# calvinmccarter/cocoa

Hardware: AMD Instinct MI355X
Metric: CoCoA+ SVM wall-clock to duality gap 1e-4; coord updates/s at 1/2/4/8 GPUs (higher is better)
Workload: dtype f64

## Files before the change

### cocoa_amd/csrc/engine.hip

```cpp
#include <hip/hip_runtime.h>

#include <sys/stat.h>
#include <unistd.h>

#include <algorithm>
#include <cerrno>
#include <cmath>
#include <cstdio>
#include <cstdlib>
#include <cstring>
#include <mutex>
#include <string>
#include <thread>
#include <vector>

#include "../../include/cocoa_capi.h"
#include "comm.h"
#include "common.h"
#include "jrandom.h"
#include "kernels.h"

using namespace cocoa;

static std::mutex g_err_mu;
// ... 192 lines not shown
    int64_t xw_stride = 0;
    hipEvent_t e_w = nullptr, e_xw = nullptr;
    bool e_w_rec = false;
    void gram_quiesce() {
        if (gstream) HIPCHK(hipStreamSynchronize(gstream));
        pre_t = -1;
    }
    hipStream_t estream = nullptr;
    hipEvent_t e_round = nullptr, e_done = nullptr;
    bool eval_pending = false;
    bool inl_pending = false;
    bool inl_since_round = false;
    bool inl_ranks = false;
    int64_t n_test_glob = -1;
    hipEvent_t e_inl = nullptr;
    cocoa_eval_result eval_held{};
    bool eval_fired = false;
    DevBuf w_snap, alpha_snap, eval_part2, eval_out2;
    DevBuf eval_cnt, eval_cnt2;
    void eval_quiesce();
    DevBuf plan_beg, plan_z, plan_zc, plan_y, plan_q, plan_xw;
    DevBuf plan_beg2, plan_z2, plan_zc2, plan_y2, plan_q2;
    bool pre_plan = false;
    DevBuf row_xw;
    bool xw_cached = false;
    Csr hot_tr, cold_tr, warm_tr;
    DevBuf hot_tiles, cold_tiles, warm_tiles, row_base;
    int64_t n_hot_tiles = 0, n_cold_tiles = 0, n_warm_tiles = 0;
    bool split_ready = false;
    Csr hot_te, cold_te;
    DevBuf hot_t_tiles, cold_t_tiles;
    int64_t n_hot_t_tiles = 0, n_cold_t_tiles = 0;
    bool te_split = false;
    DevBuf csc_ptr, csc_row, csc_val, csc_tiles, row_cnt, row_c;
    int64_t n_csc_tiles = 0;
    bool csc_ready = false;
    bool mbsgd_pull = false;
    int32_t max_z = 0;

    bool stats = false;
    uint32_t stats_mask = ~0u;
    struct Pending {
        int kid;
        hipEvent_t a, b;
    };
    std::vector<Pending> pending;
    std::vector<hipEvent_t> ev_pool;
    double tot_ms[COCOA_K_COUNT] = {0};
    int64_t cnt[COCOA_K_COUNT] = {0};

    hipEvent_t get_ev() {
        if (!ev_pool.empty()) {
            hipEvent_t e = ev_pool.back();
            ev_pool.pop_back();
            return e;
        }
        hipEvent_t e;
        HIPCHK(hipEventCreate(&e));
        return e;
    }
    template <class F>
    void timed(int kid, F&& f) {
        timed_on(stream, kid, f);
    }
    template <class F>
    void timed_on(hipStream_t st, int kid, F&& f) {
// ... 689 lines not shown
            return x.first < y.first;
        });
        int64_t a = hp[(size_t)r], b = cp[(size_t)r];
        for (const auto& cvp : tmp) {
            if (cvp.first < kEvalHot) {
                hc[(size_t)a] = (uint16_t)cvp.first;
                hv[(size_t)a++] = cvp.second;
            } else {
                cc[(size_t)b] = cvp.first;
                cv[(size_t)b++] = cvp.second;
            }
        }
    }
    ctx->hot_te = Csr{};
    ctx->cold_te = Csr{};
    ctx->hot_te.n = ctx->cold_te.n = n;
    ctx->hot_te.nnz = nh;
    ctx->cold_te.nnz = nc;
    upload(ctx->hot_te.row_ptr, hp.data(), sizeof(int64_t) * (size_t)(n + 1), s);
    upload_padded(ctx->hot_te.col16, hc.data(), sizeof(uint16_t) * (size_t)nh, s);
    upload_padded(ctx->hot_te.val, hv.data(), sizeof(double) * (size_t)nh, s);
    upload(ctx->cold_te.row_ptr, cp.data(), sizeof(int64_t) * (size_t)(n + 1), s);
    upload_padded(ctx->cold_te.col, cc.data(), sizeof(int32_t) * (size_t)nc, s);
    upload_col16(ctx->cold_te.col16, cc, nc, ctx->d, s);
    upload_padded(ctx->cold_te.val, cv.data(), sizeof(double) * (size_t)nc, s);
    int hcap = kEvalTile, ccap = kEvalTile;
    eval_split_tiles(&hcap, &ccap);
    ctx->n_hot_t_tiles = make_tiles(hp.data(), n, ctx->hot_t_tiles, s, hcap);
    ctx->n_cold_t_tiles = make_tiles(cp.data(), n, ctx->cold_t_tiles, s, ccap);
    ctx->row_base.alloc(sizeof(double) * (size_t)(ctx->tr.n + n));
    ctx->te_split = ctx->n_hot_t_tiles > 0;
}

static void set_train_impl(cocoa_ctx* ctx, bool dense_in, int32_t num_parts, const int64_t* part_ptr,
                           const int64_t* row_ptr, const int32_t* col, const double* val, const double* y,
                           int64_t n_rows, int32_t num_features, int32_t part_begin, int32_t num_parts_global) {
    require(dense_in || col != nullptr, COCOA_E_ARG, "cocoa_set_train: null column array");
    ctx->gram_quiesce();
    ctx->eval_quiesce();
    require(num_parts >= 1 && part_ptr && row_ptr && y && n_rows >= 0 && num_features >= 1, COCOA_E_ARG,
            "cocoa_set_train: bad argument");
    require(part_begin >= 0 && num_parts_global >= part_begin + num_parts, COCOA_E_ARG,
            "cocoa_set_train: bad partition range");
    require(part_ptr[0] == 0 && part_ptr[num_parts] == n_rows, COCOA_E_ARG, "part_ptr must span [0, n_rows]");
    for (int k = 0; k < num_parts; ++k) require(part_ptr[k + 1] >= part_ptr[k], COCOA_E_ARG, "part_ptr not monotone");
    if (!dense_in) check_csr(row_ptr, col, n_rows, num_features);
    const int64_t nnz = row_ptr[n_rows];
    require(val != nullptr || nnz == 0, COCOA_E_ARG, "cocoa_set_train: null value array");
    ctx->tr_dense = dense_in ? n_rows >= 1 : is_dense(row_ptr, col, n_rows, num_features);
    ctx->csc_ready = false;
    ctx->te_split = false;
    if (ctx->has_test) {
        ctx->has_test = false;
        ctx->te_dense = false;
        ctx->te.n = ctx->te.nnz = 0;
        ctx->n_t_tiles = 0;
        ctx->n_test_glob = -1;
    }
    ctx->K_loc = num_parts;
    ctx->K_glob = num_parts_global;
    ctx->part_begin = part_begin;
    ctx->d = num_features;
    ctx->tr.n = n_rows;
    ctx->tr.nnz = nnz;
    ctx->h_part_ptr.assign(part_ptr, part_ptr + num_parts + 1);
    ctx->max_nl = 0;
// ... 89 lines not shown
    ctx->tr.col_lazy = dense_in;
    if (dense_in) {
        ctx->tr.col.free();
        ctx->tr.col16.free();
    } else {
        upload_padded(ctx->tr.col, pcol.data(), sizeof(int32_t) * (size_t)nnz, s);
        upload_col16(ctx->tr.col16, pcol, nnz, num_features, s);
    }
    upload_padded(ctx->tr.val, split_classes ? pval.data() : val, sizeof(double) * (size_t)nnz, s);
    if (split_classes)
        upload(ctx->row_zc, zcv.data(), sizeof(int32_t) * kGramRuns * (size_t)n_rows, s);
    else
        ctx->row_zc.free();
    upload(ctx->tr.y, y, sizeof(double) * (size_t)n_rows, s);
    upload(ctx->sqn, sq.data(), sizeof(double) * (size_t)n_rows, s);
    upload(ctx->rowflags, fl.data(), (size_t)n_rows, s);
    upload(ctx->part_ptr, part_ptr, sizeof(int64_t) * (size_t)(num_parts + 1), s);
    ctx->n_tiles = make_tiles(row_ptr, n_rows, ctx->tiles, s, eval_tile_entries(num_features));
    if (!dense_in && !ctx->tr_dense)
        build_eval_split(ctx, row_ptr, pcol, split_classes ? pval.data() : val, n_rows, num_features, s);
    else
        ctx->split_ready = false;
    if (dense_in) {
        ctx->compact_ready = false;
        ctx->priv_ready = false;
        ctx->col_local.free();
        ctx->fptr.free();
        ctx->fpos.free();
    } else {
        build_compact(ctx, row_ptr, pcol.data(), split_classes ? pval.data() : val);
    }
    HIPCHK(hipStreamSynchronize(s));
    ctx->inited = false;
}

extern "C" int cocoa_set_test(cocoa_ctx* ctx, const int64_t* row_ptr, const int32_t* col, const double* val,
                              const double* y, int64_t n_rows) {
    CAPI_BEGIN(ctx)
    require(col != nullptr || (row_ptr && n_rows >= 0 && row_ptr[n_rows] == 0), COCOA_E_ARG,
            "cocoa_set_test: null column array");
    static const int32_t no_col = 0;
    if (!col) col = &no_col;
    if (ctx->is_group()) {
        group_set_test(ctx, false, row_ptr, col, val, y, n_rows);
        return COCOA_OK;
    }
    set_test_impl(ctx, false, row_ptr, col, val, y, n_rows);
    CAPI_END(ctx)
}

static void set_test_impl(cocoa_ctx* ctx, bool dense_in, const int64_t* row_ptr, const int32_t* col,
                          const double* val, const double* y, int64_t n_rows) {
    require(dense_in || col != nullptr, COCOA_E_ARG, "cocoa_set_test: null column array");
    ctx->eval_quiesce();
    ctx->te_split = false;
    require(ctx->d > 0, COCOA_E_STATE, "cocoa_set_test: call cocoa_set_train first");
    require(row_ptr && y && n_rows >= 0, COCOA_E_ARG, "cocoa_set_test: bad argument");
    if (!dense_in) check_csr(row_ptr, col, n_rows, ctx->d);
    const int64_t nnz = row_ptr[n_rows];
    require(val != nullptr || nnz == 0, COCOA_E_ARG, "cocoa_set_test: null value array");
    hipStream_t s = ctx->stream;
    ctx->te_dense = dense_in ? n_rows >= 1 : is_dense(row_ptr, col, n_rows, ctx->d);
    ctx->te.n = n_rows;
    ctx->te.nnz = nnz;
    upload(ctx->te.row_ptr, row_ptr, sizeof(int64_t) * (size_t)(n_rows + 1), s);
    ctx->te.col_lazy = dense_in;
    if (dense_in) {
        ctx->te.col.free();
        ctx->te.col16.free();
    } else {
        std::vector<int32_t> pcol((size_t)std::max<int64_t>(nnz, 1));
        for (int64_t q = 0; q < nnz; ++q) pcol[(size_t)q] = ctx->perm[(size_t)col[q]];
        upload_padded(ctx->te.col, pcol.data(), sizeof(int32_t) * (size_t)nnz, s);
        upload_col16(ctx->te.col16, pcol, nnz, ctx->d, s);
        build_test_split(ctx, row_ptr, pcol, val, n_rows, s);
    }
    upload_padded(ctx->te.val, val, sizeof(double) * (size_t)nnz, s);
    upload(ctx->te.y, y, sizeof(double) * (size_t)n_rows, s);
    ctx->n_t_tiles = make_tiles(row_ptr, n_rows, ctx->t_tiles, s, eval_tile_entries(ctx->d));
    HIPCHK(hipStreamSynchronize(s));
    ctx->has_test = true;
    ctx->n_test_glob = -1;
    if (ctx->inited) {
        const size_t rows = (size_t)(ctx->tr.n + ctx->te.n);
        ctx->row_scratch.alloc(sizeof(double) * std::max<size_t>(rows, 1));
    }
}

static bool is_sdca(int m) { return m == COCOA_METHOD_COCOA_PLUS || m == COCOA_METHOD_COCOA || m == COCOA_METHOD_MBCD; }
static int solver_mode(int m) {
    return m == COCOA_METHOD_COCOA_PLUS ? MODE_PLUS : m == COCOA_METHOD_COCOA ? MODE_COCOA : MODE_MBCD;
}
static int32_t wrap32(int64_t x) { return (int32_t)(uint32_t)(uint64_t)x; }

static void plan_solver(cocoa_ctx* c, int64_t vec_len, bool need_prod = true) {
    SolverArgs& a = c->sa;
    size_t off = 0;
    const size_t vec_bytes = align16(sizeof(double) * (size_t)vec_len);
    int ncu = 256;
    (void)hipDeviceGetAttribute(&ncu, hipDeviceAttributeMultiprocessorCount, c->device);
    const int want = (int)std::min<int64_t>(4, std::max<int64_t>(1, ((int64_t)c->K_loc + ncu - 1) / std::max(ncu, 1)));
    const size_t budget = want > 1 ? (kLdsMax / (size_t)want) & ~(size_t)1023 : kLdsMax;
    const double zavg = c->tr.n ? (double)c->tr.nnz / (double)c->tr.n : 0.0;
    size_t cap = zavg * 4 > (double)kStreamCap ? 2 * (size_t)kStreamCap : (size_t)kStreamCap;
    auto fixed_for = [&](size_t cp) {
        return 2 * align16(cp * 4) + 2 * align16(cp * 8) + 2 * align16(sizeof(BatchMeta)) +
               (need_prod ? align16(cp * 8) : 0) + align16(sizeof(double) * kRegChunks * 64);
    };
    while (want > 1 && cap > 512 && fixed_for(cap) > budget) cap /= 2;
    if (const char* e = std::getenv("COCOA_CHAIN_CAP"))
        cap = std::max<size_t>(256, std::min<size_t>(cap, (size_t)std::atoi(e)));
    const size_t fixed = fixed_for(cap);
    size_t avail = (want > 1 ? budget : kLdsMax) - std::min(fixed, budget);
    c->vec_lds = is_sdca(c->method) && vec_bytes <= avail && want == 1;
// ... 955 lines not shown
            e.t_val = ctx->cold_te.val.as<double>();
            e.t_tiles = ctx->cold_t_tiles.as<int64_t>();
            e.n_t_tiles = ctx->n_cold_t_tiles;
            e.th_row_ptr = ctx->hot_te.row_ptr.as<int64_t>();
            e.th_col16 = ctx->hot_te.col16.as<uint16_t>();
            e.th_val = ctx->hot_te.val.as<double>();
            e.th_tiles = ctx->hot_t_tiles.as<int64_t>();
            e.n_th_tiles = ctx->n_hot_t_tiles;
        }
        if (ctx->n_warm_tiles > 0) {
            e.m_row_ptr = ctx->warm_tr.row_ptr.as<int64_t>();
            e.m_col16 = ctx->warm_tr.col16.as<uint16_t>();
            e.m_val = ctx->warm_tr.val.as<double>();
            e.m_tiles = ctx->warm_tiles.as<int64_t>();
            e.n_m_tiles = ctx->n_warm_tiles;
        }
    }
    ctx->timed_on(st, COCOA_K_EVAL, [&] {
        if (ctx->strict)
            launch_eval_strict(e, st);
        else {
            e.row_xw = async ? nullptr : ctx->row_xw.as<double>();
            if (dense_eval) {
                launch_eval_dense(e, st);
            } else {
                DevBuf& cnt = async ? ctx->eval_cnt2 : ctx->eval_cnt;
                if (!cnt.p) cnt.alloc_zero(sizeof(unsigned), st);
                e.counter = cnt.as<unsigned>();
                e.out_host = to_host ? ctx->h_eval + (async ? 4 : 0) : nullptr;
                if (to_host && gram_status) {
                    e.status = async ? ctx->status_snap.as<int>() : ctx->status.as<int>();
                    e.status_host = (int*)(ctx->h_eval + (async ? 10 : 9));
                }
                host_done = launch_eval_fast(e, eval_fast_blocks(e.n_tiles, e.n_t_tiles), st);
            }
            ctx->xw_cached = !async;
        }
    });
    if (to_host && gram_status && !host_done)
        HIPCHK(hipMemcpyAsync(ctx->h_eval + (async ? 10 : 9), async ? ctx->status_snap.p : ctx->status.p, sizeof(int),
                              hipMemcpyDeviceToHost, st));
    ctx->status_slot[async ? 1 : 0] = to_host && gram_status;
    if (async) {
        if (!host_done)
            HIPCHK(hipMemcpyAsync(ctx->h_eval + 4, ctx->eval_out2.p, 4 * sizeof(double), hipMemcpyDeviceToHost, st));
        HIPCHK(hipEventRecord(ctx->e_done, st));
    } else if (!host_done && to_host) {
        HIPCHK(hipMemcpyAsync(ctx->h_eval, ctx->eval_out.p, 4 * sizeof(double), hipMemcpyDeviceToHost, st));
    }
}

static void check_status_slot(cocoa_ctx* ctx, int which) {
    if (!ctx->status_slot[which]) return;
    ctx->status_slot[which] = false;
    if (*(volatile int*)(ctx->h_eval + 9 + which) != 0)
        throw Error(COCOA_E_HIP, "local solver: a hand-off between the solver's waves timed out (launch aborted)");
}

struct EvalLocal {
    double hinge, alpha_sum, w2, err, n_test;
};

static EvalLocal eval_collect(cocoa_ctx* ctx) {
    HIPCHK(hipStreamSynchronize(ctx->stream));
    check_status(ctx);
    return EvalLocal{ctx->h_eval[0], ctx->h_eval[1], ctx->h_eval[2], ctx->h_eval[3],
                     (double)(ctx->has_test ? ctx->te.n : 0)};
// ... 1117 lines not shown
```

### cocoa_amd/csrc/kernels.h

```cpp
#pragma once
#include <hip/hip_runtime.h>

#include <cstdint>

namespace cocoa {

enum SolverMode : int { MODE_PLUS = 0, MODE_COCOA = 1, MODE_MBCD = 2, MODE_LSGD = 3 };

constexpr int kWave = 64;
#ifndef COCOA_RUNS
#define COCOA_RUNS 8
#endif
constexpr int kGramRuns = COCOA_RUNS;
static_assert(kGramRuns == 4 || kGramRuns == 8, "column runs");
constexpr int kGramClasses = 2;
constexpr int kProfStride = 128;
constexpr int kMetaSteps = 64;
#ifndef COCOA_REG_CHUNKS
#define COCOA_REG_CHUNKS 4
#endif
constexpr int kRegChunks = COCOA_REG_CHUNKS;
constexpr int short_row_chunks(int mode, bool strict) {
    return (strict || mode == 1) ? kRegChunks : (mode == 2 ? (kRegChunks < 2 ? kRegChunks : 2) : (kRegChunks < 3 ? kRegChunks : 3));
}
// ... 141 lines not shown
};
constexpr int kXbR = 8;

struct XwArgs {
    const int64_t* part_ptr;
    const int32_t* samples;
    const int64_t* row_ptr;
    const int32_t* col;
    const double* val;
    const double* w;
    double* xw;
    int32_t* flag;
    int64_t stride;
    int32_t K, H, nbatch, epoch;
};

struct DenseArgs {
    const double* X;
    const int64_t* part_ptr;
    const int32_t* samples;
    const double* plan_y;
    const double* plan_q;
    double* alpha;
    double* dw;
    const double* w;
    int64_t d;
    int32_t H;
    int32_t proj;
    double lam_n, inv_lam_n;
    double sigma;
    double scaling;
};

struct EvalArgs {
    const int64_t* row_ptr;
    const int32_t* col;
    const double* val;
    const double* y;
    const double* alpha;
    int64_t n;
    const int64_t* t_row_ptr;
    const int32_t* t_col;
    const double* t_val;
    const double* t_y;
    int64_t n_test;
    const double* w;
    int64_t d;
    const int64_t* part_ptr;
    const int32_t* perm;
    int32_t K;
    int32_t pad;
    const int64_t* tiles;
    int64_t n_tiles;
    const int64_t* t_tiles;
    int64_t n_t_tiles;
    double* partials;
    double* out;
    double* row_scratch;
    double* row_xw;
    const uint16_t* col16;
    const uint16_t* t_col16;
    unsigned* counter;
    double* out_host;
    const int* status;
    int* status_host;
    const int64_t* h_row_ptr;
    const uint16_t* h_col16;
    const double* h_val;
    const int64_t* h_tiles;
    int64_t n_h_tiles;
    double* row_base;
    const int64_t* m_row_ptr;
    const uint16_t* m_col16;
    const double* m_val;
    const int64_t* m_tiles;
    int64_t n_m_tiles;
    const int64_t* th_row_ptr;
    const uint16_t* th_col16;
    const double* th_val;
    const int64_t* th_tiles;
    int64_t n_th_tiles;
};
constexpr int kEvalHot = 4096;
constexpr int kEvalWarm = 65536;
void eval_split_tiles(int* hot_cap, int* cold_cap);

void launch_solver_fast(int mode, bool vec_lds, bool alpha_lds, const SolverArgs& a, int grid, size_t lds,
                        hipStream_t s);
bool launch_eval_fast(const EvalArgs& a, int blocks, hipStream_t s);
int eval_fast_blocks(int64_t n, int64_t n_test);
constexpr int64_t kEvalWideD = 65536;
int eval_tile_entries(int64_t d);
void launch_plan_fast(const PlanArgs& a, hipStream_t s);
size_t gram_solver_lds(int64_t d, int32_t* hot, bool mirror = false);
void launch_gram(const GramArgs& a, hipStream_t s);
size_t gram_seq_lds();
int gram_window_batches();
bool gram_seq_supported();
void launch_xw_produce(const XwArgs& a, hipStream_t s);
void launch_xw_gather(const int64_t* part_ptr, const int32_t* samples, int32_t H, int64_t steps,
                      const double* row_xw, double* xw, hipStream_t s);
void launch_solver_gram(int mode, const GramSolverArgs& a, int grid, hipStream_t s);
bool dense_solver_fits(int64_t d, int64_t max_nl);
bool dense_eval_fits(int64_t d);
void launch_solver_dense(int mode, const DenseArgs& a, int grid, int64_t max_nl, hipStream_t s);
void launch_eval_dense(const EvalArgs& a, hipStream_t s);

void launch_plan_strict(const PlanArgs& a, hipStream_t s);
void launch_solver_strict(int mode, bool vec_lds, bool alpha_lds, const SolverArgs& a, int grid, size_t lds,
                          hipStream_t s);
void launch_eval_strict(const EvalArgs& a, hipStream_t s);
void launch_sampler(const int64_t* part_ptr, int32_t K, int32_t seed, int32_t H, int32_t* samples,
                    const uint64_t* jump_tab, hipStream_t s);
void launch_zero(double* p, int64_t n, int blocks, hipStream_t s);
void launch_dense_cols(int32_t* col, uint16_t* col16, int64_t nnz, int32_t d, hipStream_t s);
void launch_sum_slices(double* own, const double* stage, int32_t n, int32_t r, int64_t len, hipStream_t s);
void launch_fold(const double* dw, int32_t K, int64_t d, double* dw_sum, double* w, double mult, bool apply,
                 const int32_t* inv, bool zero, hipStream_t s, const double* init = nullptr);
constexpr int64_t kFoldJ = 4096;
constexpr int64_t kFoldItem = 32768;
struct FoldTail {
    const uint32_t* tbnd;
    const uint16_t* tcol16;
// ... 35 lines not shown
```

### cocoa_amd/csrc/kernels_fast.hip

```cpp
#include <algorithm>
#include <cstdlib>

#include "kernels.h"
#include "plan_impl.h"
#include "solver_dense.h"
#include "solver_gram.h"
#include "solver_impl.h"
#include "wave.h"

namespace cocoa {

void launch_solver_fast(int mode, bool vec_lds, bool alpha_lds, const SolverArgs& a, int grid, size_t lds,
                        hipStream_t s) {
    launch_solver_impl<false>(mode, vec_lds, alpha_lds, a, grid, lds, s);
}

void launch_plan_fast(const PlanArgs& a, hipStream_t s) { launch_plan_impl<false>(a, s); }

size_t gram_solver_lds(int64_t d, int32_t* hot, bool mirror) {
    constexpr size_t kLds = 160 * 1024;
    const size_t st = mirror ? sizeof(GramSolverLdsT<kGramRuns / 2>) : sizeof(GramSolverLdsT<kGramClasses>);
    const size_t base = (st + 15) & ~(size_t)15;
    const int64_t h = std::max<int64_t>(0, std::min<int64_t>(d, (int64_t)((kLds - base) / sizeof(double)) & ~(int64_t)63));
    if (hot) *hot = (int32_t)h;
// ... 112 lines not shown
    if (!gram_hot_lds() || g.hot == 0) {
        g.mirror = 0;
        lds = (sizeof(GramSolverLdsT<kGramClasses>) + 15) & ~(size_t)15;
        g.hot = 0;
        if (mode == MODE_PLUS) launch_sg<MODE_PLUS, false>(g, grid, lds, s);
        else if (mode == MODE_COCOA) launch_sg<MODE_COCOA, false>(g, grid, lds, s);
        else if (mode == MODE_LSGD) launch_sg3<MODE_LSGD, false, false>(g, grid, lds, s);
        else launch_sg<MODE_MBCD, false>(g, grid, lds, s);
        return;
    }
    if (mode == MODE_PLUS) launch_sg<MODE_PLUS, true>(g, grid, lds, s);
    else if (mode == MODE_COCOA) launch_sg<MODE_COCOA, true>(g, grid, lds, s);
    else if (mode == MODE_LSGD) launch_sg3<MODE_LSGD, true, false>(g, grid, lds, s);
    else launch_sg<MODE_MBCD, true>(g, grid, lds, s);
}

typedef int32_t i32x4 __attribute__((ext_vector_type(4)));
typedef double f64x2 __attribute__((ext_vector_type(2)));

template <int BLOCK>
__device__ __forceinline__ double block_sum_n(double v, double* red) {
    v = wave_sum(v);
    __syncthreads();
    if ((threadIdx.x & 63) == 0) red[threadIdx.x >> 6] = v;
    __syncthreads();
    double s = 0.0;
    for (int i = 0; i < BLOCK / 64; ++i) s += red[i];
    return s;
}

typedef uint16_t u16x4 __attribute__((ext_vector_type(4)));

template <bool C16>
__device__ __forceinline__ i32x4 load_cols(const int32_t* c32, const uint16_t* c16, int64_t k) {
    if (C16) {
        const u16x4 v = __builtin_nontemporal_load((const u16x4*)(c16 + k));
        return i32x4{(int32_t)v.x, (int32_t)v.y, (int32_t)v.z, (int32_t)v.w};
    }
    return __builtin_nontemporal_load((const i32x4*)(c32 + k));
}

typedef __attribute__((address_space(1))) const double gdouble;
typedef __attribute__((address_space(3))) const double ldouble;
template <int HOT>
__device__ __forceinline__ double w_at(const double* w, const double* whot, int32_t c) {
    double x;
    if (HOT > 0 && c < HOT)
        x = ((ldouble*)whot)[c];
    else
        x = ((gdouble*)w)[c];
    return x;
}

__device__ __forceinline__ void eval_reduce(const double* partials, int blocks, double* out, double* out_host,
                                            double (*red)[4], bool sc1) {
    const int tid = threadIdx.x;
    double v[4] = {0, 0, 0, 0};
    if (tid < 256)
        for (int b = tid; b < blocks; b += 256)
            for (int i = 0; i < 4; ++i) {
                double* q = const_cast<double*>(partials) + (size_t)b * 4 + i;
                v[i] += sc1 ? __hip_atomic_load(q, __ATOMIC_RELAXED, __HIP_MEMORY_SCOPE_AGENT) : *q;
            }
    for (int i = 0; i < 4; ++i) {
        const double s = wave_sum(v[i]);
        if ((tid & 63) == 0 && tid < 256) red[i][tid >> 6] = s;
    }
    __syncthreads();
    if (tid < 4) {
        const double r = ((red[tid][0] + red[tid][1]) + red[tid][2]) + red[tid][3];
        out[tid] = r;
        if (out_host) __hip_atomic_store(out_host + tid, r, __ATOMIC_RELAXED, __HIP_MEMORY_SCOPE_SYSTEM);
    }
}

template <int TILE, int BLOCK, bool C16, int DIAGW = 0, int HOT = 0, bool BASE = false>
__global__ __launch_bounds__(BLOCK) void eval_stream_kernel(EvalArgs a) {
    constexpr int UNITS = TILE / (4 * BLOCK);
    __shared__ double prod[TILE + 4];
    __shared__ uint16_t roff[TILE + 2];
    __shared__ double red[BLOCK / 64];
    __shared__ double whot[HOT > 0 ? HOT : 1];
    __shared__ double yl[kEvalRows];
    __shared__ double bl[BASE ? kEvalRows : 1];
    const int tid = threadIdx.x;
    if (HOT > 0) {
        const int32_t h = (int32_t)min<int64_t>(HOT, a.d);
        for (int32_t j = tid; j < h; j += BLOCK) whot[j] = a.w[j];
        __syncthreads();
    }
    const int sub = tid & 15, grp = tid >> 4;
    double hinge = 0.0, err = 0.0;
    const int64_t ntiles = a.n_tiles + a.n_t_tiles;
    for (int64_t t = blockIdx.x; t < ntiles; t += gridDim.x) {
        const bool test = t >= a.n_tiles;
        const int64_t tt = test ? t - a.n_tiles : t;
        const int64_t* tl = test ? a.t_tiles : a.tiles;
        const int64_t* te = tl + (test ? a.n_t_tiles : a.n_tiles) + 1;
        const int64_t* rp = test ? a.t_row_ptr : a.row_ptr;
        const int32_t* cl = test ? a.t_col : a.col;
        const uint16_t* cl16 = test ? a.t_col16 : a.col16;
        const double* vl = test ? a.t_val : a.val;
        const double* yy = test ? a.t_y : a.y;
        const int64_t r0 = tl[tt], r1 = tl[tt + 1];
        const int64_t e0 = te[tt], e1 = te[tt + 1];
        const int64_t T = e1 - e0;
        const bool has_base = BASE && (!test || a.n_th_tiles > 0);
        const double* rb = test ? a.row_base + a.n : a.row_base;
        if (T > TILE) {
            double acc = 0.0;
            for (int64_t q = e0 + tid; q < e1; q += BLOCK) acc += vl[q] * a.w[cl[q]];
            const double dot = block_sum_n<BLOCK>(acc, red) + (has_base ? rb[r0] : 0.0);
            if (tid == 0) {
                if (!test) {
                    hinge += jmax(1 - yy[r0] * dot, 0.0);
                    if (a.row_xw) a.row_xw[r0] = dot;
                } else {
                    err += (dot * yy[r0] > 0) ? 0.0 : 1.0;
                }
            }
            continue;
        }
        const int nr = (int)(r1 - r0);
        for (int i = tid; i <= nr; i += BLOCK) {
            roff[i] = (uint16_t)(rp[r0 + i] - e0);
            if (i < nr) {
                yl[i] = yy[r0 + i];
                if (has_base) bl[i] = rb[r0 + i];
            }
        }
        const int64_t base = e0 & ~(int64_t)3;
        const int sh = (int)(e0 - base);
        const int64_t span = e1 - base;
        i32x4 c[UNITS + 1];
        f64x2 v0[UNITS + 1], v1[UNITS + 1];
#pragma unroll
        for (int u = 0; u <= UNITS; ++u) {
            const int64_t k = 4 * ((int64_t)u * BLOCK + tid);
            c[u] = i32x4{0, 0, 0, 0};
            v0[u] = f64x2{0.0, 0.0};
            v1[u] = v0[u];
            if (k < span) {
                c[u] = load_cols<C16>(cl, cl16, base + k);
                if (DIAGW == 1) c[u] &= 4095;
                if (DIAGW == 2) c[u] &= 0;
                v0[u] = __builtin_nontemporal_load((const f64x2*)(vl + base + k));
                v1[u] = __builtin_nontemporal_load((const f64x2*)(vl + base + k + 2));
            }
        }
#pragma unroll
        for (int u = 0; u <= UNITS; ++u) {
            const int64_t k = 4 * ((int64_t)u * BLOCK + tid);
            if (k < span) {
                *(f64x2*)(prod + k) = f64x2{v0[u].x * w_at<HOT>(a.w, whot, c[u].x), v0[u].y * w_at<HOT>(a.w, whot, c[u].y)};
                *(f64x2*)(prod + k + 2) = f64x2{v1[u].x * w_at<HOT>(a.w, whot, c[u].z), v1[u].y * w_at<HOT>(a.w, whot, c[u].w)};
            }
        }
        __syncthreads();
        for (int r = grp; r < nr; r += BLOCK / 16) {
            const int b = roff[r] + sh, e = roff[r + 1] + sh;
            double acc = 0.0;
            for (int q = b + sub; q < e; q += 16) acc += prod[q];
            double dot = row16_sum(acc);
            if (sub == 0) {
                if (has_base) dot += bl[r];
                if (!test) {
                    hinge += jmax(1 - yl[r] * dot, 0.0);
                    if (a.row_xw) a.row_xw[r0 + r] = dot;
                } else {
                    err += (dot * yl[r] > 0) ? 0.0 : 1.0;
                }
            }
        }
        __syncthreads();
    }
    const int64_t gt = (int64_t)blockIdx.x * BLOCK + tid;
    const int64_t gs = (int64_t)gridDim.x * BLOCK;
    double al = 0.0, w2 = 0.0;
    for (int64_t i = gt; i < a.n; i += gs) al += a.alpha[i];
    for (int64_t j = gt; j < a.d; j += gs) w2 += a.w[j] * a.w[j];
    const double s0 = block_sum_n<BLOCK>(hinge, red);
    const double s1 = block_sum_n<BLOCK>(al, red);
    const double s2 = block_sum_n<BLOCK>(w2, red);
    const double s3 = block_sum_n<BLOCK>(err, red);
// ... 62 lines not shown
        if (sub == 0) {
            if (!test) {
                hinge += jmax(1 - a.y[rr] * dot, 0.0);
                if (a.row_xw) a.row_xw[rr] = dot;
            } else {
                err += (dot * a.t_y[rr] > 0) ? 0.0 : 1.0;
            }
        }
    }
    const int64_t gt = (int64_t)blockIdx.x * 256 + tid, gs = (int64_t)gridDim.x * 256;
    double al = 0.0, w2 = 0.0;
    for (int64_t i = gt; i < a.n; i += gs) al += a.alpha[i];
    for (int64_t j = gt; j < a.d; j += gs) w2 += a.w[j] * a.w[j];
    const double s0 = block_sum_n<256>(hinge, red);
    const double s1 = block_sum_n<256>(al, red);
    const double s2 = block_sum_n<256>(w2, red);
    const double s3 = block_sum_n<256>(err, red);
    if (tid == 0) {
        double* p = a.partials + (size_t)blockIdx.x * 4;
        p[0] = s0;
        p[1] = s1;
        p[2] = s2;
        p[3] = s3;
    }
}

#endif

__global__ __launch_bounds__(256) void eval_final_kernel(const double* partials, int blocks, double* out) {
    __shared__ double red[4][4];
    eval_reduce(partials, blocks, out, nullptr, red, false);
}

int eval_fast_blocks(int64_t n_tiles, int64_t n_t_tiles) {
    int64_t b = n_tiles + n_t_tiles;
    if (b > 256 * 3) b = 256 * 3;
    return (int)(b < 1 ? 1 : b);
}

#ifdef COCOA_DIAG
static int eval_variant() {
    static int v = -1;
    if (v < 0) {
        const char* e = getenv("COCOA_EVAL_VARIANT");
        v = e ? atoi(e) : 0;
    }
    return v;
}
int eval_tile_entries(int64_t d) {
    if (const char* e = getenv("COCOA_EVAL_TILE")) return atoi(e) == 2048 ? 2048 : kEvalTile;
    if (eval_variant() >= 6 && eval_variant() <= 9) return 2048;
    return d > kEvalWideD ? 2048 : kEvalTile;
}

static bool launch_eval_diag(const EvalArgs& a, bool c16, hipStream_t s) {
    const int v = eval_variant();
    if (v == 8 || v == 9) {
        const int64_t nt = a.n_tiles + a.n_t_tiles;
        if (v == 8) {
            const int nb = (int)std::max<int64_t>(1, std::min<int64_t>(nt, 1024));
            if (c16) eval_stream_kernel<2048, 512, true><<<nb, 512, 0, s>>>(a);
            else eval_stream_kernel<2048, 512, false><<<nb, 512, 0, s>>>(a);
            eval_final_kernel<<<1, 256, 0, s>>>(a.partials, nb, a.out);
        } else {
            const int nb = (int)std::max<int64_t>(1, std::min<int64_t>(nt, 2048));
            if (c16) eval_stream_kernel<2048, 256, true><<<nb, 256, 0, s>>>(a);
            else eval_stream_kernel<2048, 256, false><<<nb, 256, 0, s>>>(a);
            eval_final_kernel<<<1, 256, 0, s>>>(a.partials, nb, a.out);
        }
        return true;
    }
#define COCOA_EVAL_C16(...)                          \
    do {                                             \
// ... 18 lines not shown
            const int n2 = (int)std::min<int64_t>(a.n_tiles + a.n_t_tiles, 512);
            COCOA_EVAL_C16((eval_stream_kernel<2048, 512, C, 0, 8192><<<n2, 512, 0, s>>>(a)));
            eval_final_kernel<<<1, 256, 0, s>>>(a.partials, n2, a.out);
        }
        return true;
    }
    if (v == 3 || v == 4) {
        const int nb = eval_fast_blocks(a.n_tiles, a.n_t_tiles);
        if (v == 3) COCOA_EVAL_C16((eval_stream_kernel<kEvalTile, 512, C, 1><<<nb, 512, 0, s>>>(a)));
        else COCOA_EVAL_C16((eval_stream_kernel<kEvalTile, 512, C, 2><<<nb, 512, 0, s>>>(a)));
        eval_final_kernel<<<1, 256, 0, s>>>(a.partials, nb, a.out);
        return true;
    }
#undef COCOA_EVAL_C16
    if (v == 1 || v == 2) {
        const int nb = 2048;
        if (v == 1) {
            if (c16) eval_rows_kernel<8, true><<<nb, 256, 0, s>>>(a);
            else eval_rows_kernel<8, false><<<nb, 256, 0, s>>>(a);
        } else {
            if (c16) eval_rows_kernel<4, true><<<nb, 256, 0, s>>>(a);
            else eval_rows_kernel<4, false><<<nb, 256, 0, s>>>(a);
        }
        eval_final_kernel<<<1, 256, 0, s>>>(a.partials, nb, a.out);
        return true;
    }
    return false;
}
#else
int eval_tile_entries(int64_t d) { return d > kEvalWideD ? 2048 : kEvalTile; }
#endif

template <int TILE, int BLOCK, int HOT, bool WARM = false>
__global__ __launch_bounds__(BLOCK) void eval_hot_kernel(EvalArgs a) {
    constexpr int UNITS = TILE / (4 * BLOCK);
    __shared__ double prod[TILE + 4];
    __shared__ uint16_t roff[TILE + 2];
    __shared__ double red[BLOCK / 64];
    __shared__ double whot[WARM ? 1 : HOT];
    __shared__ double bl[WARM ? kEvalRows : 1];
    const int tid = threadIdx.x;
    if (!WARM) {
        const int32_t h = (int32_t)min<int64_t>(HOT, a.d);
        for (int32_t j = tid; j < HOT; j += BLOCK) whot[j] = j < h ? a.w[j] : 0.0;
        __syncthreads();
    }
    const gdouble* wm = (const gdouble*)(a.w + kEvalHot);
    auto w_of = [&](int32_t c) -> double { return WARM ? wm[c] : whot[c]; };
    const int sub = tid & 15, grp = tid >> 4;
    const int64_t nt = WARM ? a.n_m_tiles : a.n_h_tiles;
    const int64_t ntt = WARM ? 0 : a.n_th_tiles;
    for (int64_t t = blockIdx.x; t < nt + ntt; t += gridDim.x) {
        const bool test = t >= nt;
        const int64_t tt = test ? t - nt : t;
        const int64_t* tl = test ? a.th_tiles : WARM ? a.m_tiles : a.h_tiles;
        const int64_t* te = tl + (test ? ntt : nt) + 1;
        const int64_t* rp = test ? a.th_row_ptr : WARM ? a.m_row_ptr : a.h_row_ptr;
        const uint16_t* cl = test ? a.th_col16 : WARM ? a.m_col16 : a.h_col16;
        const double* vl = test ? a.th_val : WARM ? a.m_val : a.h_val;
        double* rb = test ? a.row_base + a.n : a.row_base;
        const int64_t r0 = tl[tt], r1 = tl[tt + 1];
        const int64_t e0 = te[tt], e1 = te[tt + 1];
        const int64_t T = e1 - e0;
        if (T > TILE) {
            double acc = 0.0;
            for (int64_t q = e0 + tid; q < e1; q += BLOCK) acc += vl[q] * w_of(cl[q]);
            const double dot = block_sum_n<BLOCK>(acc, red);
            if (tid == 0) rb[r0] = WARM ? rb[r0] + dot : dot;
            continue;
        }
        const int nr = (int)(r1 - r0);
        for (int i = tid; i <= nr; i += BLOCK) {
            roff[i] = (uint16_t)(rp[r0 + i] - e0);
            if (WARM && i < nr) bl[i] = rb[r0 + i];
        }
        const int64_t base = e0 & ~(int64_t)3;
        const int sh = (int)(e0 - base);
        const int64_t span = e1 - base;
        i32x4 c[UNITS + 1];
        f64x2 v0[UNITS + 1], v1[UNITS + 1];
#pragma unroll
        for (int u = 0; u <= UNITS; ++u) {
            const int64_t k = 4 * ((int64_t)u * BLOCK + tid);
            c[u] = i32x4{0, 0, 0, 0};
            v0[u] = f64x2{0.0, 0.0};
            v1[u] = v0[u];
            if (k < span) {
                c[u] = load_cols<true>(nullptr, cl, base + k);
                v0[u] = __builtin_nontemporal_load((const f64x2*)(vl + base + k));
                v1[u] = __builtin_nontemporal_load((const f64x2*)(vl + base + k + 2));
            }
        }
#pragma unroll
        for (int u = 0; u <= UNITS; ++u) {
            const int64_t k = 4 * ((int64_t)u * BLOCK + tid);
            if (k < span) {
                *(f64x2*)(prod + k) = f64x2{v0[u].x * w_of(c[u].x), v0[u].y * w_of(c[u].y)};
                *(f64x2*)(prod + k + 2) = f64x2{v1[u].x * w_of(c[u].z), v1[u].y * w_of(c[u].w)};
            }
        }
        __syncthreads();
        for (int r = grp; r < nr; r += BLOCK / 16) {
            const int b = roff[r] + sh, e = roff[r + 1] + sh;
            double acc = 0.0;
            for (int q = b + sub; q < e; q += 16) acc += prod[q];
            const double dot = row16_sum(acc);
            if (sub == 0) rb[r0 + r] = WARM ? bl[r] + dot : dot;
        }
        __syncthreads();
    }
}

#ifndef COCOA_HOT_TILE
#define COCOA_HOT_TILE 4096
#endif
#ifndef COCOA_HOT_BLOCK
#define COCOA_HOT_BLOCK 1024
#endif
#ifndef COCOA_HOT_WGS
#define COCOA_HOT_WGS 2
#endif
#ifndef COCOA_COLD_TILE
#define COCOA_COLD_TILE 4096
#endif
#ifndef COCOA_COLD_BLOCK
#define COCOA_COLD_BLOCK 512
#endif
void eval_split_tiles(int* hot_cap, int* cold_cap) {
    *hot_cap = COCOA_HOT_TILE;
    *cold_cap = COCOA_COLD_TILE;
}

template <typename F>
static int resident_grid(F kernel, int threads, int want) {
    int per_cu = 0, dev = 0, cus = 256;
    (void)hipGetDevice(&dev);
    (void)hipDeviceGetAttribute(&cus, hipDeviceAttributeMultiprocessorCount, dev);
    if (hipOccupancyMaxActiveBlocksPerMultiprocessor(&per_cu, kernel, threads, 0) != hipSuccess || per_cu < 1) {
        (void)hipGetLastError();
        return want;
    }
    return std::max(1, std::min(want, per_cu * cus));
}

static bool launch_eval_split(const EvalArgs& a, int blocks, hipStream_t s) {
    const bool c16 = a.col16 && (a.n_test == 0 || a.t_col16);
    const int hb = (int)std::max<int64_t>(1, std::min<int64_t>(a.n_h_tiles + a.n_th_tiles, 256 * COCOA_HOT_WGS));
    eval_hot_kernel<COCOA_HOT_TILE, COCOA_HOT_BLOCK, kEvalHot><<<hb, COCOA_HOT_BLOCK, 0, s>>>(a);
    if (a.n_m_tiles > 0) {
        const int mb = resident_grid(eval_hot_kernel<COCOA_HOT_TILE, COCOA_HOT_BLOCK, kEvalHot, true>, COCOA_HOT_BLOCK,
                                     (int)std::max<int64_t>(1, std::min<int64_t>(a.n_m_tiles, 256 * 8)));
        eval_hot_kernel<COCOA_HOT_TILE, COCOA_HOT_BLOCK, kEvalHot, true><<<mb, COCOA_HOT_BLOCK, 0, s>>>(a);
    }
    if (c16) {
        blocks = resident_grid(eval_stream_kernel<COCOA_COLD_TILE, COCOA_COLD_BLOCK, true, 0, 0, true>, COCOA_COLD_BLOCK,
                               blocks);
        eval_stream_kernel<COCOA_COLD_TILE, COCOA_COLD_BLOCK, true, 0, 0, true><<<blocks, COCOA_COLD_BLOCK, 0, s>>>(a);
    } else {
        blocks = resident_grid(eval_stream_kernel<COCOA_COLD_TILE, COCOA_COLD_BLOCK, false, 0, 0, true>,
                               COCOA_COLD_BLOCK, blocks);
        eval_stream_kernel<COCOA_COLD_TILE, COCOA_COLD_BLOCK, false, 0, 0, true><<<blocks, COCOA_COLD_BLOCK, 0, s>>>(a);
    }
    if (!a.counter) eval_final_kernel<<<1, 256, 0, s>>>(a.partials, blocks, a.out);
    return a.counter && a.out_host;
}

bool launch_eval_fast(const EvalArgs& a, int blocks, hipStream_t s) {
    if (a.row_base) return launch_eval_split(a, blocks, s);
    const bool c16 = a.col16 && (a.n_test == 0 || a.t_col16);
#ifdef COCOA_DIAG
    EvalArgs u = a;
    u.counter = nullptr;
    if (launch_eval_diag(u, c16, s)) return false;
#endif
    if (c16) {
        blocks = resident_grid(eval_stream_kernel<kEvalTile, 512, true>, 512, blocks);
        eval_stream_kernel<kEvalTile, 512, true><<<blocks, 512, 0, s>>>(a);
    } else if (a.d > kEvalWideD) {
        blocks = resident_grid(eval_stream_kernel<2048, 512, false, 0, 4096>, 512, blocks);
        eval_stream_kernel<2048, 512, false, 0, 4096><<<blocks, 512, 0, s>>>(a);
    } else {
        blocks = resident_grid(eval_stream_kernel<kEvalTile, 512, false>, 512, blocks);
        eval_stream_kernel<kEvalTile, 512, false><<<blocks, 512, 0, s>>>(a);
    }
    if (!a.counter) eval_final_kernel<<<1, 256, 0, s>>>(a.partials, blocks, a.out);
    return a.counter && a.out_host;
}

template <bool TAIL>
__global__ __launch_bounds__(256) void fold_blocks_kernel(const double* dw, const uint16_t* fcol16,
                                                          const uint32_t* fbnd, const int32_t* items, int32_t K,
                                                          int64_t max_u, int64_t d, double* tmp, FoldTail tl) {
    constexpr int kUn = 4;
    __shared__ double acc[kFoldJ];
    const int tid = threadIdx.x, lane = tid & 63, wv = tid >> 6;
    const int32_t* it = items + 4 * (size_t)blockIdx.x;
    const int32_t b = it[0], k0 = it[1], k1 = it[2], sole = it[3];
    for (int i = tid; i < kFoldJ; i += 256) acc[i] = 0.0;
    __syncthreads();
    for (int part = 0; part < (TAIL ? 2 : 1); ++part) {
        const uint32_t* bnd = part ? tl.tbnd : fbnd;
        for (int32_t kk = k0; kk < k1; kk += 64) {
            const int32_t k = kk + lane;
            const bool ok = k < k1;
            const int32_t lo = ok ? (int32_t)bnd[(size_t)b * K + k] : 0;
            const int32_t n = ok ? (int32_t)bnd[(size_t)(b + 1) * K + k] - lo : 0;
            const int32_t incl = wave_incl_scan(n);
            const int32_t T = __shfl(incl, 63, 64);
            const int32_t excl = incl - n;
            for (int32_t q0 = 64 * kUn * wv; q0 < T; q0 += 64 * kUn * 4) {
                size_t pos[kUn];
                bool val[kUn];
#pragma unroll
                for (int u = 0; u < kUn; ++u) {
                    const int32_t q = q0 + 64 * u + lane;
                    int j = 0;
#pragma unroll
// ... 292 lines not shown
```

Baseline: 348.6 million.

## Software-pipeline hot eval tiles and precompute eval launch grids at setup

The hot/warm eval kernel now prefetches the next tile's row offsets, columns and values into registers while the current tile is reduced. Tile bounds are fetched with four lanes and broadcast via readlane, and 16-bit columns stay narrow until use. Occupancy-based grid sizes for all eval kernels are computed once when train or test data is set, so per-eval occupancy and device queries are gone. The cost is more register pressure (a launch-bounds hint is added), a smaller hot tile cap, and a cached grid that could go stale if the device or data changes.

```diff
diff --git a/cocoa_amd/csrc/engine.hip b/cocoa_amd/csrc/engine.hip
--- a/cocoa_amd/csrc/engine.hip
+++ b/cocoa_amd/csrc/engine.hip
@@ -248,6 +248,7 @@
     DevBuf hot_t_tiles, cold_t_tiles;
     int64_t n_hot_t_tiles = 0, n_cold_t_tiles = 0;
     bool te_split = false;
+    EvalGrids eval_g{};
     DevBuf csc_ptr, csc_row, csc_val, csc_tiles, row_cnt, row_c;
     int64_t n_csc_tiles = 0;
     bool csc_ready = false;
@@ -1003,6 +1004,13 @@
     ctx->te_split = ctx->n_hot_t_tiles > 0;
 }
 
+static void plan_eval_grids(cocoa_ctx* ctx) {
+    const int64_t tt = ctx->has_test ? ctx->n_t_tiles : 0;
+    const bool ts = ctx->has_test && ctx->te_split;
+    ctx->eval_g = eval_grids(ctx->n_tiles + tt, ctx->n_cold_tiles + (ts ? ctx->n_cold_t_tiles : tt),
+                             ctx->n_hot_tiles + (ts ? ctx->n_hot_t_tiles : 0), ctx->n_warm_tiles, ctx->d);
+}
+
 static void set_train_impl(cocoa_ctx* ctx, bool dense_in, int32_t num_parts, const int64_t* part_ptr,
                            const int64_t* row_ptr, const int32_t* col, const double* val, const double* y,
                            int64_t n_rows, int32_t num_features, int32_t part_begin, int32_t num_parts_global) {
@@ -1158,6 +1166,7 @@
     }
     HIPCHK(hipStreamSynchronize(s));
     ctx->inited = false;
+    plan_eval_grids(ctx);
 }
 
 extern "C" int cocoa_set_test(cocoa_ctx* ctx, const int64_t* row_ptr, const int32_t* col, const double* val,
@@ -1206,6 +1215,7 @@
     ctx->n_t_tiles = make_tiles(row_ptr, n_rows, ctx->t_tiles, s, eval_tile_entries(ctx->d));
     HIPCHK(hipStreamSynchronize(s));
     ctx->has_test = true;
+    plan_eval_grids(ctx);
     ctx->n_test_glob = -1;
     if (ctx->inited) {
         const size_t rows = (size_t)(ctx->tr.n + ctx->te.n);
@@ -2227,7 +2237,8 @@
                     e.status = async ? ctx->status_snap.as<int>() : ctx->status.as<int>();
                     e.status_host = (int*)(ctx->h_eval + (async ? 10 : 9));
                 }
-                host_done = launch_eval_fast(e, eval_fast_blocks(e.n_tiles, e.n_t_tiles), st);
+                e.g = ctx->eval_g;
+                host_done = launch_eval_fast(e, st);
             }
             ctx->xw_cached = !async;
         }
diff --git a/cocoa_amd/csrc/kernels.h b/cocoa_amd/csrc/kernels.h
--- a/cocoa_amd/csrc/kernels.h
+++ b/cocoa_amd/csrc/kernels.h
@@ -197,6 +197,9 @@
     double scaling;
 };
 
+struct EvalGrids {
+    int32_t one[2], cold[2], hot, warm;
+};
 struct EvalArgs {
     const int64_t* row_ptr;
     const int32_t* col;
@@ -245,6 +248,7 @@
     const double* th_val;
     const int64_t* th_tiles;
     int64_t n_th_tiles;
+    EvalGrids g;
 };
 constexpr int kEvalHot = 4096;
 constexpr int kEvalWarm = 65536;
@@ -252,8 +256,8 @@
 
 void launch_solver_fast(int mode, bool vec_lds, bool alpha_lds, const SolverArgs& a, int grid, size_t lds,
                         hipStream_t s);
-bool launch_eval_fast(const EvalArgs& a, int blocks, hipStream_t s);
-int eval_fast_blocks(int64_t n, int64_t n_test);
+bool launch_eval_fast(const EvalArgs& a, hipStream_t s);
+EvalGrids eval_grids(int64_t one_tiles, int64_t cold_tiles, int64_t hot_tiles, int64_t warm_tiles, int64_t d);
 constexpr int64_t kEvalWideD = 65536;
 int eval_tile_entries(int64_t d);
 void launch_plan_fast(const PlanArgs& a, hipStream_t s);
diff --git a/cocoa_amd/csrc/kernels_fast.hip b/cocoa_amd/csrc/kernels_fast.hip
--- a/cocoa_amd/csrc/kernels_fast.hip
+++ b/cocoa_amd/csrc/kernels_fast.hip
@@ -168,12 +168,45 @@
 typedef uint16_t u16x4 __attribute__((ext_vector_type(4)));
 
 template <bool C16>
-__device__ __forceinline__ i32x4 load_cols(const int32_t* c32, const uint16_t* c16, int64_t k) {
-    if (C16) {
-        const u16x4 v = __builtin_nontemporal_load((const u16x4*)(c16 + k));
-        return i32x4{(int32_t)v.x, (int32_t)v.y, (int32_t)v.z, (int32_t)v.w};
-    }
-    return __builtin_nontemporal_load((const i32x4*)(c32 + k));
+struct ColVec {
+    typedef i32x4 type;
+};
+template <>
+struct ColVec<true> {
+    typedef u16x4 type;
+};
+template <bool C16>
+__device__ __forceinline__ typename ColVec<C16>::type load_cols(const int32_t* c32, const uint16_t* c16, int64_t k) {
+    if constexpr (C16)
+        return __builtin_nontemporal_load((const u16x4*)(c16 + k));
+    else
+        return __builtin_nontemporal_load((const i32x4*)(c32 + k));
+}
+__device__ __forceinline__ i32x4 widen_cols(u16x4 v) { return i32x4{(int32_t)v.x, (int32_t)v.y, (int32_t)v.z, (int32_t)v.w}; }
+__device__ __forceinline__ i32x4 widen_cols(i32x4 v) { return v; }
+
+__device__ __forceinline__ int64_t tile_bounds(const int64_t* tl, int64_t ntl, int64_t tt) {
+    const int i = threadIdx.x & 3;
+    return tl[tt + (i & 1) + (i >> 1) * (ntl + 1)];
+}
+__device__ __forceinline__ int64_t lane_i64(int64_t v, int lane) {
+    const uint32_t lo = (uint32_t)__builtin_amdgcn_readlane((int)v, lane);
+    const uint32_t hi = (uint32_t)__builtin_amdgcn_readlane((int)(v >> 32), lane);
+    return (int64_t)(((uint64_t)hi << 32) | lo);
+}
+struct EvalTile {
+    int64_t r0, e0, e1;
+    int nr;
+    bool test;
+};
+__device__ __forceinline__ EvalTile tile_of(int64_t raw, bool test) {
+    EvalTile x;
+    x.r0 = lane_i64(raw, 0);
+    x.nr = (int)(lane_i64(raw, 1) - x.r0);
+    x.e0 = lane_i64(raw, 2);
+    x.e1 = lane_i64(raw, 3);
+    x.test = test;
+    return x;
 }
 
 typedef __attribute__((address_space(1))) const double gdouble;
@@ -212,9 +245,9 @@
 
 template <int TILE, int BLOCK, bool C16, int DIAGW = 0, int HOT = 0, bool BASE = false>
 __global__ __launch_bounds__(BLOCK) void eval_stream_kernel(EvalArgs a) {
-    constexpr int UNITS = TILE / (4 * BLOCK);
+    constexpr int UNITS = TILE / (4 * BLOCK) + 1;
     __shared__ double prod[TILE + 4];
-    __shared__ uint16_t roff[TILE + 2];
+    __shared__ uint16_t roff[kEvalRows + 2];
     __shared__ double red[BLOCK / 64];
     __shared__ double whot[HOT > 0 ? HOT : 1];
     __shared__ double yl[kEvalRows];
@@ -268,16 +301,16 @@
         const int64_t base = e0 & ~(int64_t)3;
         const int sh = (int)(e0 - base);
         const int64_t span = e1 - base;
-        i32x4 c[UNITS + 1];
-        f64x2 v0[UNITS + 1], v1[UNITS + 1];
-#pragma unroll
-        for (int u = 0; u <= UNITS; ++u) {
+        i32x4 c[UNITS];
+        f64x2 v0[UNITS], v1[UNITS];
+#pragma unroll
+        for (int u = 0; u < UNITS; ++u) {
             const int64_t k = 4 * ((int64_t)u * BLOCK + tid);
             c[u] = i32x4{0, 0, 0, 0};
             v0[u] = f64x2{0.0, 0.0};
             v1[u] = v0[u];
             if (k < span) {
-                c[u] = load_cols<C16>(cl, cl16, base + k);
+                c[u] = widen_cols(load_cols<C16>(cl, cl16, base + k));
                 if (DIAGW == 1) c[u] &= 4095;
                 if (DIAGW == 2) c[u] &= 0;
                 v0[u] = __builtin_nontemporal_load((const f64x2*)(vl + base + k));
@@ -285,7 +318,7 @@
             }
         }
 #pragma unroll
-        for (int u = 0; u <= UNITS; ++u) {
+        for (int u = 0; u < UNITS; ++u) {
             const int64_t k = 4 * ((int64_t)u * BLOCK + tid);
             if (k < span) {
                 *(f64x2*)(prod + k) = f64x2{v0[u].x * w_at<HOT>(a.w, whot, c[u].x), v0[u].y * w_at<HOT>(a.w, whot, c[u].y)};
@@ -414,13 +447,13 @@
     eval_reduce(partials, blocks, out, nullptr, red, false);
 }
 
-int eval_fast_blocks(int64_t n_tiles, int64_t n_t_tiles) {
+#ifdef COCOA_DIAG
+static int eval_fast_blocks(int64_t n_tiles, int64_t n_t_tiles) {
     int64_t b = n_tiles + n_t_tiles;
     if (b > 256 * 3) b = 256 * 3;
     return (int)(b < 1 ? 1 : b);
 }
 
-#ifdef COCOA_DIAG
 static int eval_variant() {
     static int v = -1;
     if (v < 0) {
@@ -505,10 +538,11 @@
 #endif
 
 template <int TILE, int BLOCK, int HOT, bool WARM = false>
-__global__ __launch_bounds__(BLOCK) void eval_hot_kernel(EvalArgs a) {
+__global__ __launch_bounds__(BLOCK, (BLOCK == 1024 ? 8 : 1)) void eval_hot_kernel(EvalArgs a) {
     constexpr int UNITS = TILE / (4 * BLOCK);
-    __shared__ double prod[TILE + 4];
-    __shared__ uint16_t roff[TILE + 2];
+    constexpr int RI = (kEvalRows + BLOCK - 1) / BLOCK;
+    __shared__ double prod[TILE];
+    __shared__ uint16_t roff[kEvalRows + 2];
     __shared__ double red[BLOCK / 64];
     __shared__ double whot[WARM ? 1 : HOT];
     __shared__ double bl[WARM ? kEvalRows : 1];
@@ -523,54 +557,107 @@
     const int sub = tid & 15, grp = tid >> 4;
     const int64_t nt = WARM ? a.n_m_tiles : a.n_h_tiles;
     const int64_t ntt = WARM ? 0 : a.n_th_tiles;
-    for (int64_t t = blockIdx.x; t < nt + ntt; t += gridDim.x) {
-        const bool test = t >= nt;
-        const int64_t tt = test ? t - nt : t;
-        const int64_t* tl = test ? a.th_tiles : WARM ? a.m_tiles : a.h_tiles;
-        const int64_t* te = tl + (test ? ntt : nt) + 1;
-        const int64_t* rp = test ? a.th_row_ptr : WARM ? a.m_row_ptr : a.h_row_ptr;
+    const int64_t ntot = nt + ntt, G = gridDim.x;
+    if ((int64_t)blockIdx.x >= ntot) return;
+    constexpr bool PIPE = !WARM;
+    auto bounds = [&](int64_t t) __attribute__((always_inline)) {
+        return t >= nt ? tile_bounds(a.th_tiles, ntt, t - nt) : tile_bounds(WARM ? a.m_tiles : a.h_tiles, nt, t);
+    };
+    u16x4 c[UNITS];
+    f64x2 v0[UNITS], v1[UNITS];
+    uint32_t ro[RI];
+    double bv[WARM ? RI : 1];
+    auto issue = [&](const EvalTile& x) __attribute__((always_inline)) {
+        const int64_t base = x.e0 & ~(int64_t)3;
+        const int64_t span = x.e1 - base;
+        if (span > TILE) return;
+        const int64_t* rp = x.test ? a.th_row_ptr : WARM ? a.m_row_ptr : a.h_row_ptr;
+        const uint16_t* cl = x.test ? a.th_col16 : WARM ? a.m_col16 : a.h_col16;
+        const double* vl = x.test ? a.th_val : WARM ? a.m_val : a.h_val;
+        const double* rb = x.test ? a.row_base + a.n : a.row_base;
+#pragma unroll
+        for (int j = 0; j < RI; ++j) {
+            const int i = tid + j * BLOCK;
+            ro[j] = 0;
+            if (WARM) bv[j] = 0.0;
+            if (i < x.nr) ro[j] = (uint32_t)rp[x.r0 + i];
+            if (WARM && i < x.nr) bv[j] = rb[x.r0 + i];
+        }
+#pragma unroll
+        for (int u = 0; u < UNITS; ++u) {
+            const int64_t k = 4 * ((int64_t)u * BLOCK + tid);
+            c[u] = u16x4{0, 0, 0, 0};
+            v0[u] = f64x2{0.0, 0.0};
+            v1[u] = v0[u];
+            if (k < span) {
+                c[u] = load_cols<true>(nullptr, cl, base + k);
+                v0[u] = __builtin_nontemporal_load((const f64x2*)(vl + base + k));
+                v1[u] = __builtin_nontemporal_load((const f64x2*)(vl + base + k + 2));
+            }
+        }
+    };
+    EvalTile nx{};
+    int64_t braw = 0;
+    if (PIPE) {
+        nx = tile_of(bounds(blockIdx.x), (int64_t)blockIdx.x >= nt);
+        issue(nx);
+        if (blockIdx.x + G < ntot) braw = bounds(blockIdx.x + G);
+    }
+    for (int64_t t = blockIdx.x; t < ntot; t += G) {
+        if (!PIPE) {
+            nx = tile_of(bounds(t), t >= nt);
+            issue(nx);
+        }
+        vm_drain();
+        const EvalTile x = nx;
+        const bool more = PIPE && t + G < ntot;
+        if (PIPE) nx = tile_of(braw, t + G >= nt);
+        const bool test = x.test;
         const uint16_t* cl = test ? a.th_col16 : WARM ? a.m_col16 : a.h_col16;
         const double* vl = test ? a.th_val : WARM ? a.m_val : a.h_val;
         double* rb = test ? a.row_base + a.n : a.row_base;
-        const int64_t r0 = tl[tt], r1 = tl[tt + 1];
-        const int64_t e0 = te[tt], e1 = te[tt + 1];
+        const int64_t r0 = x.r0, e0 = x.e0, e1 = x.e1;
         const int64_t T = e1 - e0;
+        const int nr = x.nr;
+        const int64_t base = e0 & ~(int64_t)3;
+        int sh = (int)(e0 - base);
+        const int64_t span = e1 - base;
+        if (span <= TILE) {
+#pragma unroll
+            for (int j = 0; j < RI; ++j) {
+                const int i = tid + j * BLOCK;
+                if (i < nr) roff[i] = (uint16_t)(ro[j] - (uint32_t)e0);
+                if (WARM && i < nr) bl[i] = bv[j];
+            }
+            if (tid == 0) roff[nr] = (uint16_t)T;
+#pragma unroll
+            for (int u = 0; u < UNITS; ++u) {
+                const int64_t k = 4 * ((int64_t)u * BLOCK + tid);
+                if (k < span) {
+                    const i32x4 cc = widen_cols(c[u]);
+                    *(f64x2*)(prod + k) = f64x2{v0[u].x * w_of(cc.x), v0[u].y * w_of(cc.y)};
+                    *(f64x2*)(prod + k + 2) = f64x2{v1[u].x * w_of(cc.z), v1[u].y * w_of(cc.w)};
+                }
+            }
+        } else if (T <= TILE) {
+            for (int k = tid; k < (int)T; k += BLOCK) prod[k] = vl[e0 + k] * w_of(cl[e0 + k]);
+            if (tid == 0) {
+                roff[0] = 0;
+                roff[1] = (uint16_t)T;
+                if (WARM) bl[0] = rb[r0];
+            }
+            sh = 0;
+        }
+        if (more) {
+            issue(nx);
+            if (t + 2 * G < ntot) braw = bounds(t + 2 * G);
+        }
         if (T > TILE) {
             double acc = 0.0;
             for (int64_t q = e0 + tid; q < e1; q += BLOCK) acc += vl[q] * w_of(cl[q]);
             const double dot = block_sum_n<BLOCK>(acc, red);
             if (tid == 0) rb[r0] = WARM ? rb[r0] + dot : dot;
             continue;
-        }
-        const int nr = (int)(r1 - r0);
-        for (int i = tid; i <= nr; i += BLOCK) {
-            roff[i] = (uint16_t)(rp[r0 + i] - e0);
-            if (WARM && i < nr) bl[i] = rb[r0 + i];
-        }
-        const int64_t base = e0 & ~(int64_t)3;
-        const int sh = (int)(e0 - base);
-        const int64_t span = e1 - base;
-        i32x4 c[UNITS + 1];
-        f64x2 v0[UNITS + 1], v1[UNITS + 1];
-#pragma unroll
-        for (int u = 0; u <= UNITS; ++u) {
-            const int64_t k = 4 * ((int64_t)u * BLOCK + tid);
-            c[u] = i32x4{0, 0, 0, 0};
-            v0[u] = f64x2{0.0, 0.0};
-            v1[u] = v0[u];
-            if (k < span) {
-                c[u] = load_cols<true>(nullptr, cl, base + k);
-                v0[u] = __builtin_nontemporal_load((const f64x2*)(vl + base + k));
-                v1[u] = __builtin_nontemporal_load((const f64x2*)(vl + base + k + 2));
-            }
-        }
-#pragma unroll
-        for (int u = 0; u <= UNITS; ++u) {
-            const int64_t k = 4 * ((int64_t)u * BLOCK + tid);
-            if (k < span) {
-                *(f64x2*)(prod + k) = f64x2{v0[u].x * w_of(c[u].x), v0[u].y * w_of(c[u].y)};
-                *(f64x2*)(prod + k + 2) = f64x2{v1[u].x * w_of(c[u].z), v1[u].y * w_of(c[u].w)};
-            }
         }
         __syncthreads();
         for (int r = grp; r < nr; r += BLOCK / 16) {
@@ -600,62 +687,74 @@
 #define COCOA_COLD_BLOCK 512
 #endif
 void eval_split_tiles(int* hot_cap, int* cold_cap) {
-    *hot_cap = COCOA_HOT_TILE;
+    *hot_cap = COCOA_HOT_TILE - 3;
     *cold_cap = COCOA_COLD_TILE;
 }
 
 template <typename F>
-static int resident_grid(F kernel, int threads, int want) {
-    int per_cu = 0, dev = 0, cus = 256;
-    (void)hipGetDevice(&dev);
-    (void)hipDeviceGetAttribute(&cus, hipDeviceAttributeMultiprocessorCount, dev);
+static int resident_grid(F kernel, int threads, int cus, int64_t want) {
+    int per_cu = 0;
+    want = std::max<int64_t>(1, want);
     if (hipOccupancyMaxActiveBlocksPerMultiprocessor(&per_cu, kernel, threads, 0) != hipSuccess || per_cu < 1) {
         (void)hipGetLastError();
-        return want;
-    }
-    return std::max(1, std::min(want, per_cu * cus));
-}
-
-static bool launch_eval_split(const EvalArgs& a, int blocks, hipStream_t s) {
+        return (int)std::min<int64_t>(want, 3 * (int64_t)cus);
+    }
+    return (int)std::min<int64_t>(want, (int64_t)per_cu * cus);
+}
+
+EvalGrids eval_grids(int64_t one_tiles, int64_t cold_tiles, int64_t hot_tiles, int64_t warm_tiles, int64_t d) {
+    int dev = 0, cus = 256;
+    (void)hipGetDevice(&dev);
+    if (hipDeviceGetAttribute(&cus, hipDeviceAttributeMultiprocessorCount, dev) != hipSuccess || cus < 1) {
+        (void)hipGetLastError();
+        cus = 256;
+    }
+    EvalGrids g{};
+    const int64_t one = std::min<int64_t>(one_tiles, 3 * (int64_t)cus);
+    g.one[1] = resident_grid(eval_stream_kernel<kEvalTile, 512, true>, 512, cus, one);
+    g.one[0] = d > kEvalWideD ? resident_grid(eval_stream_kernel<2048, 512, false, 0, 4096>, 512, cus, one)
+                              : resident_grid(eval_stream_kernel<kEvalTile, 512, false>, 512, cus, one);
+    const int64_t cold = std::min<int64_t>(cold_tiles, 3 * (int64_t)cus);
+    g.cold[1] = resident_grid(eval_stream_kernel<COCOA_COLD_TILE, COCOA_COLD_BLOCK, true, 0, 0, true>, COCOA_COLD_BLOCK,
+                              cus, cold);
+    g.cold[0] = resident_grid(eval_stream_kernel<COCOA_COLD_TILE, COCOA_COLD_BLOCK, false, 0, 0, true>, COCOA_COLD_BLOCK,
+                              cus, cold);
+    g.hot = resident_grid(eval_hot_kernel<COCOA_HOT_TILE, COCOA_HOT_BLOCK, kEvalHot>, COCOA_HOT_BLOCK, cus,
+                          std::min<int64_t>(hot_tiles, (int64_t)cus * COCOA_HOT_WGS));
+    g.warm = resident_grid(eval_hot_kernel<COCOA_HOT_TILE, COCOA_HOT_BLOCK, kEvalHot, true>, COCOA_HOT_BLOCK, cus,
+                           std::min<int64_t>(warm_tiles, (int64_t)cus * 8));
+    return g;
+}
+
+static bool launch_eval_split(const EvalArgs& a, hipStream_t s) {
     const bool c16 = a.col16 && (a.n_test == 0 || a.t_col16);
-    const int hb = (int)std::max<int64_t>(1, std::min<int64_t>(a.n_h_tiles + a.n_th_tiles, 256 * COCOA_HOT_WGS));
-    eval_hot_kernel<COCOA_HOT_TILE, COCOA_HOT_BLOCK, kEvalHot><<<hb, COCOA_HOT_BLOCK, 0, s>>>(a);
-    if (a.n_m_tiles > 0) {
-        const int mb = resident_grid(eval_hot_kernel<COCOA_HOT_TILE, COCOA_HOT_BLOCK, kEvalHot, true>, COCOA_HOT_BLOCK,
-                                     (int)std::max<int64_t>(1, std::min<int64_t>(a.n_m_tiles, 256 * 8)));
-        eval_hot_kernel<COCOA_HOT_TILE, COCOA_HOT_BLOCK, kEvalHot, true><<<mb, COCOA_HOT_BLOCK, 0, s>>>(a);
-    }
-    if (c16) {
-        blocks = resident_grid(eval_stream_kernel<COCOA_COLD_TILE, COCOA_COLD_BLOCK, true, 0, 0, true>, COCOA_COLD_BLOCK,
-                               blocks);
+    eval_hot_kernel<COCOA_HOT_TILE, COCOA_HOT_BLOCK, kEvalHot><<<a.g.hot, COCOA_HOT_BLOCK, 0, s>>>(a);
+    if (a.n_m_tiles > 0)
+        eval_hot_kernel<COCOA_HOT_TILE, COCOA_HOT_BLOCK, kEvalHot, true><<<a.g.warm, COCOA_HOT_BLOCK, 0, s>>>(a);
+    const int blocks = a.g.cold[c16];
+    if (c16)
         eval_stream_kernel<COCOA_COLD_TILE, COCOA_COLD_BLOCK, true, 0, 0, true><<<blocks, COCOA_COLD_BLOCK, 0, s>>>(a);
-    } else {
-        blocks = resident_grid(eval_stream_kernel<COCOA_COLD_TILE, COCOA_COLD_BLOCK, false, 0, 0, true>,
-                               COCOA_COLD_BLOCK, blocks);
+    else
         eval_stream_kernel<COCOA_COLD_TILE, COCOA_COLD_BLOCK, false, 0, 0, true><<<blocks, COCOA_COLD_BLOCK, 0, s>>>(a);
-    }
     if (!a.counter) eval_final_kernel<<<1, 256, 0, s>>>(a.partials, blocks, a.out);
     return a.counter && a.out_host;
 }
 
-bool launch_eval_fast(const EvalArgs& a, int blocks, hipStream_t s) {
-    if (a.row_base) return launch_eval_split(a, blocks, s);
+bool launch_eval_fast(const EvalArgs& a, hipStream_t s) {
+    if (a.row_base) return launch_eval_split(a, s);
     const bool c16 = a.col16 && (a.n_test == 0 || a.t_col16);
 #ifdef COCOA_DIAG
     EvalArgs u = a;
     u.counter = nullptr;
     if (launch_eval_diag(u, c16, s)) return false;
 #endif
-    if (c16) {
-        blocks = resident_grid(eval_stream_kernel<kEvalTile, 512, true>, 512, blocks);
+    const int blocks = a.g.one[c16];
+    if (c16)
         eval_stream_kernel<kEvalTile, 512, true><<<blocks, 512, 0, s>>>(a);
-    } else if (a.d > kEvalWideD) {
-        blocks = resident_grid(eval_stream_kernel<2048, 512, false, 0, 4096>, 512, blocks);
+    else if (a.d > kEvalWideD)
         eval_stream_kernel<2048, 512, false, 0, 4096><<<blocks, 512, 0, s>>>(a);
-    } else {
-        blocks = resident_grid(eval_stream_kernel<kEvalTile, 512, false>, 512, blocks);
+    else
         eval_stream_kernel<kEvalTile, 512, false><<<blocks, 512, 0, s>>>(a);
-    }
     if (!a.counter) eval_final_kernel<<<1, 256, 0, s>>>(a.partials, blocks, a.out);
     return a.counter && a.out_host;
 }
```

New measurement: 349.3 million (median of 6 runs). No clear change (+0.2%).
